# LowLevelAI/GLARE

Hardware: AMD Instinct MI355X
Metric: enhanced images/sec (400x600) (higher is better)
Workload: dtype fp16; 1 GPU; LOL eval15-shaped 400x600 inference, batch=8 per GPU, full encoder->flow->VQ->decoder->AFT (BASELINE configs[1]); batch_per_gpu=8, global_batch=8, input=3x400x600 (reflect-padded to 420x620), parallelism=dp1, streams_per_gpu=2, exchange=none (1 GPU), ranks_seen=1, weights=random, name-seeded (no checkpoints offline)

## Files before the change

glare_amd/csrc/conv_igemm_kernel.h:

```cpp
#pragma once
#include <type_traits>

#include "common.h"



struct ConvParams {
  const a16_t* in0;
  const a16_t* in1;
  const a16_t* wpk;
  const float* bias;
  const a16_t* res;
  void* out;
  int B, H, W;
  int IHs, IWs;
  int OH, OW;
  int Cin0, Cin1, CinTot;
  int p0, o0, p1, o1;
  int Cout, opitch, ooff, rpitch, roff;
  int upsample, act, out_mode;
  long long plane_pitch;
  int tiles_x, tiles_y, co_tiles, n_blocks, n_stages;
  int fast_epilogue;
  unsigned in0_bytes, in1_bytes;
  unsigned res_bytes;
  float* gn_part;
  int gn_nparts;
  const a16_t* res_lo;
  a16_t* out_lo;
  int groups, g_in_step, g_out_step, g_bias_step;
  long long g_w_elems;
  int k_wrap;
  const float* gn_coef;
  int gn_swish;
};

enum { EPI_FAST = 0,
       EPI_PLANAR = 1,
       EPI_GENERAL = 2 };
__host__ inline int conv_pick_epilogue(const ConvParams& p, bool planar_kernel) {
  const bool expk = p.act == GLARE_ACT_SIGMOID || p.act == GLARE_ACT_SWISH;
  if (p.out_mode == GLARE_OUT_NHWC_BF16 && p.fast_epilogue && !(p.res == nullptr && expk)) return EPI_FAST;
  if (planar_kernel && p.out_mode == GLARE_OUT_PLANAR_F32 && !p.res && !expk) return EPI_PLANAR;
  return EPI_GENERAL;
}

int glare_conv_launch_k3s1(const ConvParams& p, int tn, bool hilo, hipStream_t stream);
int glare_conv_launch_k3s1_planar(const ConvParams& p, int tn, hipStream_t stream);
int glare_conv_launch_k3s1_general(const ConvParams& p, int tn, hipStream_t stream);
int glare_conv_launch_k3s2(const ConvParams& p, int tn, bool hilo, hipStream_t stream);
int glare_conv_launch_k3s2_general(const ConvParams& p, int tn, hipStream_t stream);
int glare_conv_launch_k1(const ConvParams& p, int tn, bool hilo, hipStream_t stream);
int glare_conv_launch_k1_general(const ConvParams& p, int tn, hipStream_t stream);
int glare_conv_launch_k2(const ConvParams& p, int tn, hipStream_t stream);

namespace {

constexpr int TW = 32;



template <int KS, int STRIDE, int TH>
struct TileGeom {
  static constexpr int IH = (TH - 1) * STRIDE + KS;
  static constexpr int IW = (TW - 1) * STRIDE + KS;
  static constexpr int NPOS = IH * IW;
  static constexpr int PAD = (KS == 3 && STRIDE == 1) ? 1 : 0;
};

template <int N, typename F>
__device__ __forceinline__ void static_for(F&& f) {
  if constexpr (N > 0) {
    static_for<N - 1>(f);
    f(std::integral_constant<int, N - 1>{});
  }
}



__device__ __forceinline__ int fresh_lane_id() {
  int l;
  asm volatile("v_mbcnt_lo_u32_b32 %0, -1, 0\n\tv_mbcnt_hi_u32_b32 %0, -1, %0" : "=v"(l));
  return l;
}

__device__ __forceinline__ void gn_prologue_piece(u32x4* slot, const float* cf, int swish) {
  __builtin_amdgcn_sched_barrier(0);
  u32x4 v = *slot;
#pragma unroll
  for (int e = 0; e < 4; ++e) {
    const f32x4 q = *reinterpret_cast<const f32x4*>(cf + 4 * e);
    float lo = alo(v[e]) * q[0] + q[1];
    float hi = ahi(v[e]) * q[2] + q[3];
    if (swish) { lo = swishf_(lo); hi = swishf_(hi); }
    v[e] = pack_a2(lo, hi);
    __builtin_amdgcn_sched_barrier(0);
  }
  *slot = v;
  __builtin_amdgcn_sched_barrier(0);
}

template <int KS, int STRIDE, int MT, int NT, int WM, int WN, int KSTEPS, bool HILO = false, bool GNP = false, int EPI = EPI_FAST>
__global__ __launch_bounds__(64 * WM * WN, ((STRIDE == 1 && WM * WN == 4) ? 3 : 2)) void conv_igemm_kernel(const ConvParams p_in) {
  ConvParams p = p_in;
  if (p.groups > 1) {
    const int g = blockIdx.y;
    p.o0 += g * p.g_in_step;
    p.o1 += g * p.g_in_step;
    p.ooff += g * p.g_out_step;
    p.wpk += (size_t)g * p.g_w_elems;
    if (p.bias) p.bias += g * p.g_bias_step;
  }
  constexpr int TH = WM * MT;
  constexpr int NW = WM * WN;
  using G = TileGeom<KS, STRIDE, TH>;
  static_assert(NW == 4 || NW == 6 || NW == 8, "wave layout");
  constexpr int TN = WN * NT * 32;
  constexpr int A_CHUNKS = KSTEPS * 2 * G::NPOS;
  constexpr int A_INSTR = (A_CHUNKS + 63) / 64;
  constexpr int A_SLOTS = A_INSTR * 64;
  constexpr int A_PER_W = (A_INSTR + NW - 1) / NW;
  constexpr int B_CHUNKS = KS * KSTEPS * 2 * TN;
  static_assert(B_CHUNKS % 64 == 0, "B stage is a whole number of wave DMAs");
  constexpr int B_INSTR = B_CHUNKS / 64;
  constexpr int B_PER_W = (B_INSTR + NW - 1) / NW;
  constexpr int KC = 16 * KSTEPS;

  extern __shared__ __attribute__((aligned(16))) char smem[];
  u32x4* lA = reinterpret_cast<u32x4*>(smem);
  u32x4* lB = lA + 2 * A_SLOTS;

  int bid = blockIdx.x;
  {
    const int n = p.n_blocks, q = n / 8, r = n % 8, xcd = bid % 8, k = bid / 8;
    bid = (xcd < r ? xcd * (q + 1) : r * (q + 1) + (xcd - r) * q) + k;
  }
  const int ct = bid % p.co_tiles;
  int t = bid / p.co_tiles;
  int phase = 0;
  if (KS == 2) { phase = t & 3; t >>= 2; }
  const int pa = phase >> 1, pb = phase & 1;
  const int tx = t % p.tiles_x;
  t /= p.tiles_x;
  const int ty = t % p.tiles_y;
  const int b = t / p.tiles_y;

  const int tid = threadIdx.x, lane = tid & 63;
  const int wave = __builtin_amdgcn_readfirstlane(tid >> 6);
  const int wm = wave / WN, wn = wave % WN;
  const int oy0 = ty * TH, ox0 = tx * TW;
  const int iy0 = oy0 * STRIDE - G::PAD - (KS == 2 ? 1 - pa : 0), ix0 = ox0 * STRIDE - G::PAD - (KS == 2 ? 1 - pb : 0);

  f32x16 acc[MT][NT];
#pragma unroll
  for (int i = 0; i < MT; ++i)
#pragma unroll
    for (int j = 0; j < NT; ++j)
#pragma unroll
      for (int r = 0; r < 16; ++r) acc[i][j][r] = 0.f;

  constexpr unsigned A_OOB = 0x80000000u;
  unsigned a_vo0[A_PER_W], a_vo1[A_PER_W];
  int a_ck[A_PER_W];
#pragma unroll
  for (int i = 0; i < A_PER_W; ++i) {
    const int c = (wave + NW * i) * 64 + lane;
    a_vo0[i] = a_vo1[i] = A_OOB;
    a_ck[i] = 0;
    if (c < A_CHUNKS) {
      const int prow = c / (2 * KSTEPS * G::IW), rem = c % (2 * KSTEPS * G::IW);
      const int kk = rem / G::IW, pos = prow * G::IW + rem % G::IW;
      a_ck[i] = kk * 8;
      const int iy = iy0 + pos / G::IW, ix = ix0 + pos % G::IW;
      if (iy >= 0 && iy < p.IHs && ix >= 0 && ix < p.IWs) {
        const int sy = p.upsample ? (iy >> 1) : iy, sx = p.upsample ? (ix >> 1) : ix;
        const unsigned pix = (unsigned)(sy * p.W + sx);
        a_vo0[i] = (pix * (unsigned)p.p0 + (unsigned)(p.o0 + kk * 8)) * 2u;
        if constexpr (!GNP) a_vo1[i] = (pix * (unsigned)p.p1 + (unsigned)(p.o1 + kk * 8)) * 2u;
      }
    }
  }
  const size_t img = (size_t)b * p.H * p.W;
  const __amdgpu_buffer_rsrc_t arsrc0 =
      __builtin_amdgcn_make_buffer_rsrc(const_cast<a16_t*>(p.in0 + img * p.p0), 0, (int)p.in0_bytes, 0x00020000);
  const __amdgpu_buffer_rsrc_t arsrc1 = __builtin_amdgcn_make_buffer_rsrc(
      const_cast<a16_t*>(p.in1 ? p.in1 + img * p.p1 : p.in0), 0, (int)(p.in1 ? p.in1_bytes : p.in0_bytes), 0x00020000);
  const a16_t* wbase = p.wpk + ((size_t)phase * p.co_tiles + ct) * p.n_stages * (size_t)(KS * B_CHUNKS) * 8;

  const bool reuse = KS == 3 && !GNP && p.k_wrap == 2;
  const int n_pair = reuse ? 2 * (p.Cin0 / KC) : 0;
  auto a_is_new = [&](int stage) { return !(reuse && stage < n_pair && (stage & 1)); };
  auto issue_a = [&](int chunk, int buf, int i_lo = 0, int i_hi = 1 << 20) {
    const int c0 = chunk * KC;
    bool src0 = GNP || c0 < p.Cin0 || c0 >= p.Cin0 + p.Cin1;
    int cbase = c0 < p.Cin0 ? c0 : (src0 ? c0 - p.Cin0 - p.Cin1 : c0 - p.Cin0);
    if (reuse) {
      src0 = chunk < n_pair;
      cbase = src0 ? (chunk >> 1) * KC : (chunk - n_pair) * KC;
    }
    const int climit = src0 ? p.Cin0 : p.Cin1;
#pragma unroll
    for (int i = 0; i < A_PER_W; ++i) {
      const int j = wave + NW * i;
      if (i >= i_lo && i < i_hi && j < A_INSTR) {
        unsigned vo = src0 ? a_vo0[i] : a_vo1[i];
        if (cbase + a_ck[i] >= climit) vo = A_OOB;
        if (src0)
          __builtin_amdgcn_raw_ptr_buffer_load_lds(arsrc0, (__attribute__((address_space(3))) void*)(lA + buf * A_SLOTS + j * 64), 16, vo,
                                                   cbase * 2, 0, 0);
        else
          __builtin_amdgcn_raw_ptr_buffer_load_lds(arsrc1, (__attribute__((address_space(3))) void*)(lA + buf * A_SLOTS + j * 64), 16, vo,
                                                   cbase * 2, 0, 0);
      }
    }
  };
  const __amdgpu_buffer_rsrc_t wrsrc = __builtin_amdgcn_make_buffer_rsrc(
      const_cast<a16_t*>(wbase), 0, (int)((size_t)p.n_stages * KS * B_CHUNKS * 16), 0x00020000);
  const int lane16 = lane * 16;
  auto issue_b = [&](int bstage, int buf, int i_lo = 0, int i_hi = 1 << 20) {
#pragma unroll
    for (int i = 0; i < B_PER_W; ++i) {
      const int j = wave + NW * i;
      if (i >= i_lo && i < i_hi && j < B_INSTR)
        __builtin_amdgcn_raw_ptr_buffer_load_lds(wrsrc, (__attribute__((address_space(3))) void*)(lB + buf * B_CHUNKS + j * 64),
                                                 16, lane16, (bstage * B_CHUNKS + j * 64) * 16, 0, 0);
    }
  };

  [[maybe_unused]] auto prefetch_residual = [&](int free_buf) {
    if constexpr (KS == 3 && STRIDE == 1 && NW == 4 && TN == 128) {
      static_assert(A_SLOTS * 16 >= NW * 4 * 256, "room for the prefetch's landing zone");
      const size_t rimg = (size_t)b * p.OH * p.OW * p.rpitch;
#pragma unroll
      for (int k = 0; k < 2; ++k) {
        const int l = (wave * 2 + k) * 64 + lane;
        const int oy = oy0 + (l >> 6), ox = ox0 + ((l >> 1) & 31), co = ct * TN + (l & 1) * 64;
        const unsigned vo = (oy < p.OH && ox < p.OW && co < p.Cout)
                                ? (unsigned)(((oy * p.OW + ox) * p.rpitch + p.roff + co) * 2) : 0x80000000u;
        const __amdgpu_buffer_rsrc_t rr = __builtin_amdgcn_make_buffer_rsrc(const_cast<a16_t*>(p.res + rimg), 0, (int)p.res_bytes, 0x00020000);
        __builtin_amdgcn_raw_ptr_buffer_load_lds(rr, (__attribute__((address_space(3))) void*)(lA + free_buf * A_SLOTS + (wave * 4 + k) * 16),
                                                 4, vo, 0, 0, 0);
        if constexpr (HILO) {
          if (p.res_lo) {
            const __amdgpu_buffer_rsrc_t rl =
                __builtin_amdgcn_make_buffer_rsrc(const_cast<a16_t*>(p.res_lo + rimg), 0, (int)p.res_bytes, 0x00020000);
            __builtin_amdgcn_raw_ptr_buffer_load_lds(rl, (__attribute__((address_space(3))) void*)(lA + free_buf * A_SLOTS + (wave * 4 + 2 + k) * 16),
                                                     4, vo, 0, 0, 0);
          }
        }
      }
    }
  };

  [[maybe_unused]] float* lC = reinterpret_cast<float*>(lB + 2 * B_CHUNKS);
  [[maybe_unused]] auto gn_transform = [&](int chunk, int buf) {
    if constexpr (GNP) {
      const int c0 = chunk * KC;
#pragma unroll
      for (int i = 0; i < A_PER_W; ++i) {
        const int j = wave + NW * i;
        if (j < A_INSTR && a_vo0[i] != A_OOB && c0 + a_ck[i] < p.Cin0) {
          int ln = fresh_lane_id(), ck = a_ck[i];
          asm volatile("" : "+v"(ln), "+v"(ck));
          gn_prologue_piece(lA + buf * A_SLOTS + j * 64 + ln, lC + (c0 + ck) * 2, p.gn_swish);
        }
      }
    }
  };
  if constexpr (GNP) {
    const float* src = p.gn_coef + (size_t)b * p.Cin0 * 2;
    for (int i = tid; i < p.Cin0 * 2; i += 64 * NW) lC[i] = src[i];
    __syncthreads();
  }

  const int khalf = lane >> 5, px = lane & 31;
  const int n_bstages = p.n_stages * KS;
  issue_a(0, 0);
  issue_b(0, 0);
  int bs = 0;
  int a_cnt = 0;
  for (int chunk = 0; chunk < p.n_stages; ++chunk) {
    const u32x4* cA = lA + (a_cnt & 1) * A_SLOTS;
    const bool next_new = chunk + 1 < p.n_stages && a_is_new(chunk + 1);
#pragma unroll
    for (int trow = 0; trow < KS; ++trow, ++bs) {
      asm volatile("s_waitcnt vmcnt(0)" ::: "memory");
      if constexpr (GNP) {
        if (trow == 0 && chunk == 0) gn_transform(0, 0);
        if (trow == 1 && chunk + 1 < p.n_stages) gn_transform(chunk + 1, (a_cnt + 1) & 1);
      }
      __syncthreads();
      constexpr int NGRP = KS * KSTEPS;
      [[maybe_unused]] constexpr int B_PG = (B_PER_W + NGRP - 1) / NGRP, A_PG = (A_PER_W + NGRP - 1) / NGRP;
      const bool more_b = bs + 1 < n_bstages, more_a = trow == 0 && next_new;
      if (trow == 0 && chunk + 1 == p.n_stages && p.res_bytes) prefetch_residual((a_cnt + 1) & 1);
      const u32x4* cB = lB + (bs & 1) * B_CHUNKS;
#pragma unroll
      for (int tcol = 0; tcol < KS; ++tcol) {
#pragma unroll
        for (int ks = 0; ks < KSTEPS; ++ks) {
          {
            const int grp = tcol * KSTEPS + ks;
            if (more_b) issue_b(bs + 1, (bs + 1) & 1, grp * B_PG, (grp + 1) * B_PG);
            if (more_a) issue_a(chunk + 1, (a_cnt + 1) & 1, grp * A_PG, (grp + 1) * A_PG);
          }
          a16x8 bf[NT], af[MT];
#pragma unroll
          for (int j = 0; j < NT; ++j) {
            const int co = (wn * NT + j) * 32 + px;
            bf[j] = __builtin_bit_cast(a16x8, cB[((tcol * KSTEPS + ks) * 2 + khalf) * TN + co]);
          }
#pragma unroll
          for (int i = 0; i < MT; ++i) {
            const int row = wm * MT + i;
            af[i] = __builtin_bit_cast(a16x8, cA[((row * STRIDE + trow) * (2 * KSTEPS) + ks * 2 + khalf) * G::IW + px * STRIDE + tcol]);
          }
#pragma unroll
          for (int i = 0; i < MT; ++i)
#pragma unroll
            for (int j = 0; j < NT; ++j)
              acc[i][j] = mfma_a16_32x32x16(af[i], bf[j], acc[i][j], 0, 0, 0);
        }
      }
    }
    if (next_new) ++a_cnt;
  }

  if constexpr (HILO) {
    constexpr int ROWF = NT * 128 + 16;
    constexpr int CPR = NT * 4;
    static_assert(NW * 32 * ROWF <= (2 * A_SLOTS + 2 * B_CHUNKS) * 16, "hi/lo epilogue slab fits the pipeline LDS");
    static_assert(KS != 2, "the sub-pixel form has no hi/lo epilogue");
    __syncthreads();
    char* slab = smem + wave * (32 * ROWF);
    const int lane = fresh_lane_id();
    const int ncol = lane & 31, rhalf = lane >> 5;
    float gs0 = 0.f, gq0 = 0.f, gs1 = 0.f, gq1 = 0.f;
    const ActSel asel = act_sel(p.act);
    static_for<MT>([&](auto ic) {
      constexpr int i = decltype(ic)::value;
      static_for<NT>([&](auto jc) {
        constexpr int j = decltype(jc)::value;
        const int co = ct * TN + (wn * NT + j) * 32 + ncol;
        const float bv = (p.bias && co < p.Cout) ? p.bias[co] : 0.f;
#pragma unroll
        for (int r = 0; r < 16; ++r) {
          const int m = (r & 3) + 8 * (r >> 2) + 4 * rhalf;
          *reinterpret_cast<float*>(slab + m * ROWF + (j * 32 + ncol) * 4) = acc[i][j][r] + bv;
        }
      });
      constexpr int NIT = 32 * CPR / 64;
      [[maybe_unused]] u32x4 rvv[NIT], rlv[NIT];
      const bool res_buf = p.res && p.res_bytes;
      __builtin_amdgcn_sched_barrier(0);
      if (res_buf) {
        const size_t rimg = (size_t)b * p.OH * p.OW * p.rpitch;
        const __amdgpu_buffer_rsrc_t rr = __builtin_amdgcn_make_buffer_rsrc(const_cast<a16_t*>(p.res + rimg), 0, (int)p.res_bytes, 0x00020000);
        const __amdgpu_buffer_rsrc_t rl = __builtin_amdgcn_make_buffer_rsrc(const_cast<a16_t*>((p.res_lo ? p.res_lo : p.res) + rimg), 0,
                                                                            (int)p.res_bytes, 0x00020000);
        const int oy = oy0 + wm * MT + i;
        const unsigned vo = oy < p.OH ? (unsigned)((((oy * p.OW + ox0 + lane / CPR) * p.rpitch) + p.roff + ct * TN + wn * NT * 32 + (lane % CPR) * 8) * 2)
                                      : 0x80000000u;
#pragma unroll
        for (int it = 0; it < NIT; ++it) {
          const unsigned o = vo + (unsigned)(it * (64 / CPR) * p.rpitch * 2);
          rvv[it] = __builtin_amdgcn_raw_buffer_load_b128(rr, o, 0, 0);
          if (p.res_lo) rlv[it] = __builtin_amdgcn_raw_buffer_load_b128(rl, o, 0, 0);
        }
      }
      asm volatile("s_waitcnt lgkmcnt(0)" ::: "memory");
#pragma unroll
      for (int it = 0; it < NIT; ++it) {
        const int idx = lane + 64 * it;
        const int row = idx / CPR, ch = idx % CPR;
        const int oy = oy0 + wm * MT + i, ox = ox0 + row;
        const int co = ct * TN + wn * NT * 32 + ch * 8;
        if (oy < p.OH && ox < p.OW && co < p.Cout) {
          const f32x4 f0 = *reinterpret_cast<const f32x4*>(slab + row * ROWF + ch * 32);
          const f32x4 f1 = *reinterpret_cast<const f32x4*>(slab + row * ROWF + ch * 32 + 16);
          float v[8] = {f0[0], f0[1], f0[2], f0[3], f1[0], f1[1], f1[2], f1[3]};
          const size_t pix = ((size_t)b * p.OH + oy) * p.OW + ox;
          if (p.res) {
            const u32x4 rv = res_buf ? rvv[it] : *reinterpret_cast<const u32x4*>(p.res + pix * p.rpitch + p.roff + co);
#pragma unroll
            for (int e = 0; e < 4; ++e) { v[2 * e] += alo(rv[e]); v[2 * e + 1] += ahi(rv[e]); }
            if (p.res_lo) {
              const u32x4 rl = res_buf ? rlv[it] : *reinterpret_cast<const u32x4*>(p.res_lo + pix * p.rpitch + p.roff + co);
#pragma unroll
              for (int e = 0; e < 4; ++e) { v[2 * e] += alo(rl[e]); v[2 * e + 1] += ahi(rl[e]); }
            }
          }
          if (asel.expk) {
#pragma unroll
            for (int e = 0; e < 8; ++e) v[e] = act_exp(v[e], asel.expk);
          } else {
#pragma unroll
            for (int e = 0; e < 8; ++e) v[e] = act_cheap(v[e], asel.relu);
          }
          u32x4 hi, lo;
#pragma unroll
          for (int e = 0; e < 4; ++e) {
            const float a = v[2 * e], c = v[2 * e + 1];
            hi[e] = pack_a2(a, c);
            lo[e] = pack_a2(a - alo(hi[e]), c - ahi(hi[e]));
            if (e < 2) { gs0 += a + c; gq0 += a * a + c * c; } else { gs1 += a + c; gq1 += a * a + c * c; }
          }
          *reinterpret_cast<u32x4*>(reinterpret_cast<a16_t*>(p.out) + pix * p.opitch + p.ooff + co) = hi;
          *reinterpret_cast<u32x4*>(p.out_lo + pix * p.opitch + p.ooff + co) = lo;
        }
      }
      asm volatile("s_waitcnt lgkmcnt(0)" ::: "memory");
    });
    if (p.gn_part) {
#pragma unroll
      for (int o = CPR; o < 64; o <<= 1) {
        gs0 += __shfl_xor(gs0, o, 64); gq0 += __shfl_xor(gq0, o, 64);
        gs1 += __shfl_xor(gs1, o, 64); gq1 += __shfl_xor(gq1, o, 64);
      }
      const int co = ct * TN + wn * NT * 32 + lane * 8;
      if (lane < CPR && co < p.Cout) {
        const int row0 = oy0 + wm * MT;
        const int part = ((phase * ((p.OH + 7) / 8) + row0 / 8) * p.tiles_x + tx) * 2 + ((row0 / 4) & 1);
        if (part < p.gn_nparts) {
          float* dst = p.gn_part + (((size_t)b * p.gn_nparts + part) * (p.Cout / 4) + co / 4) * 2;
          dst[0] = gs0; dst[1] = gq0; dst[2] = gs1; dst[3] = gq1;
        }
      }
    }
    return;
  }

  if constexpr (EPI == EPI_FAST) {
    constexpr int HT = (NW == 8 || MT < 2) ? 1 : MT / 2;
    constexpr int HROWS = HT * 32;
    constexpr int ROWB = NT * 64 + 16;
    constexpr int CPR = NT * 4;
    static_assert(NW * HROWS * ROWB <= (2 * A_SLOTS + 2 * B_CHUNKS) * 16, "epilogue slab fits the pipeline LDS");
    __syncthreads();
    char* slab = smem + wave * (HROWS * ROWB);
    const int lane = fresh_lane_id();
    const int ncol = lane & 31, rhalf = lane >> 5, odd = lane & 1;
    const bool act_early = p.res == nullptr;
    float gs0 = 0.f, gq0 = 0.f, gs1 = 0.f, gq1 = 0.f;
    const ActSel asel = act_sel(p.act);
    const bool relu_early = act_early && asel.relu;
    static_for<MT / HT>([&](auto hc) {
      constexpr int half = decltype(hc)::value;
      static_for<NT>([&](auto jc) {
        constexpr int j = decltype(jc)::value;
        const int co = ct * TN + (wn * NT + j) * 32 + ncol;
        const float bv = (p.bias && co < p.Cout) ? p.bias[co] : 0.f;
        static_for<HT>([&](auto ic) {
          constexpr int il = decltype(ic)::value;
#pragma unroll
          for (int t = 0; t < 8; ++t) {
            constexpr int i = half * HT + il;
            const float a = act_cheap(acc[i][j][2 * t] + bv, relu_early), c = act_cheap(acc[i][j][2 * t + 1] + bv, relu_early);
            const float send = odd ? a : c;
            const float recv = __shfl_xor(send, 1, 64);
            const int r = 2 * t + odd;
            const int m = (r & 3) + 8 * (r >> 2) + 4 * rhalf;
            const uint32_t w = odd ? pack_a2(recv, c) : pack_a2(a, recv);
            *reinterpret_cast<uint32_t*>(slab + (il * 32 + m) * ROWB + (j * 32 + (ncol & ~1)) * 2) = w;
          }
        });
      });
      constexpr int NIT = HROWS * CPR / 64;
      constexpr bool RES_AHEAD = NIT <= 8 && KS != 2;
      [[maybe_unused]] u32x4 rvv[RES_AHEAD ? NIT : 1];
      bool res_buf = false;
      if constexpr (RES_AHEAD) {
        res_buf = p.res && p.res_bytes;
        __builtin_amdgcn_sched_barrier(0);
        if (res_buf) {
          const size_t rimg = (size_t)b * p.OH * p.OW * p.rpitch;
          const __amdgpu_buffer_rsrc_t rr = __builtin_amdgcn_make_buffer_rsrc(const_cast<a16_t*>(p.res + rimg), 0, (int)p.res_bytes, 0x00020000);
          const int oyb = oy0 + wm * MT + half * HT;
          const unsigned vo = (unsigned)((((oyb * p.OW + ox0 + lane / CPR) * p.rpitch) + p.roff + ct * TN + wn * NT * 32 + (lane % CPR) * 8) * 2);
#pragma unroll
          for (int it = 0; it < NIT; ++it) {
            constexpr int RPI = 64 / CPR;
            const int dy = (it * RPI) / 32, dx = (it * RPI) % 32;
            const unsigned o = oyb + dy < p.OH ? vo + (unsigned)((dy * p.OW + dx) * p.rpitch * 2) : 0x80000000u;
            rvv[it] = __builtin_amdgcn_raw_buffer_load_b128(rr, o, 0, 0);
          }
        }
      }
      asm volatile("s_waitcnt lgkmcnt(0)" ::: "memory");
#pragma unroll
      for (int it = 0; it < NIT; ++it) {
        const int idx = lane + 64 * it;
        const int row = idx / CPR, ch = idx % CPR;
        const int oy = oy0 + wm * MT + half * HT + row / 32, ox = ox0 + (row & 31);
        const int co = ct * TN + wn * NT * 32 + ch * 8;
        if (oy < p.OH && ox < p.OW && co < p.Cout) {
          u32x4 v = *reinterpret_cast<const u32x4*>(slab + row * ROWB + ch * 16);
          const size_t pix = KS == 2 ? ((size_t)b * (2 * p.OH) + 2 * oy + pa) * (size_t)(2 * p.OW) + 2 * ox + pb
                                     : ((size_t)b * p.OH + oy) * p.OW + ox;
          if (p.res) {
            u32x4 rv;
            if (res_buf) rv = rvv[RES_AHEAD ? it : 0];
            else rv = *reinterpret_cast<const u32x4*>(p.res + pix * p.rpitch + p.roff + co);
            if (asel.expk) {
#pragma unroll
              for (int e = 0; e < 4; ++e) v[e] = pack_a2(act_exp(alo(v[e]) + alo(rv[e]), asel.expk), act_exp(ahi(v[e]) + ahi(rv[e]), asel.expk));
            } else {
#pragma unroll
              for (int e = 0; e < 4; ++e) v[e] = pack_a2(act_cheap(alo(v[e]) + alo(rv[e]), asel.relu), act_cheap(ahi(v[e]) + ahi(rv[e]), asel.relu));
            }
          }
          *reinterpret_cast<u32x4*>(reinterpret_cast<a16_t*>(p.out) + pix * p.opitch + p.ooff + co) = v;
          if (p.gn_part) {
#pragma unroll
            for (int e = 0; e < 2; ++e) {
              const float x0 = alo(v[e]), x1 = ahi(v[e]), y0 = alo(v[2 + e]), y1 = ahi(v[2 + e]);
              gs0 += x0 + x1; gq0 += x0 * x0 + x1 * x1;
              gs1 += y0 + y1; gq1 += y0 * y0 + y1 * y1;
            }
          }
        }
      }
      asm volatile("s_waitcnt lgkmcnt(0)" ::: "memory");
    });
    if (p.gn_part) {
#pragma unroll
      for (int o = CPR; o < 64; o <<= 1) {
        gs0 += __shfl_xor(gs0, o, 64); gq0 += __shfl_xor(gq0, o, 64);
        gs1 += __shfl_xor(gs1, o, 64); gq1 += __shfl_xor(gq1, o, 64);
      }
      const int co = ct * TN + wn * NT * 32 + lane * 8;
      if (lane < CPR && co < p.Cout) {
        const int row0 = oy0 + wm * MT;
        const int part = ((phase * ((p.OH + 7) / 8) + row0 / 8) * p.tiles_x + tx) * 2 + ((row0 / 4) & 1);
        if (part < p.gn_nparts) {
          float* dst = p.gn_part + (((size_t)b * p.gn_nparts + part) * (p.Cout / 4) + co / 4) * 2;
          dst[0] = gs0; dst[1] = gq0; dst[2] = gs1; dst[3] = gq1;
        }
      }
    }
    return;
  }

  if constexpr (EPI == EPI_PLANAR) {
    static_assert(!HILO && KS == 3 && STRIDE == 1 && NW == 4, "the planar slab epilogue exists for the 3x3 stride-1 4-wave kernels");
    {
      constexpr int ROWD = NT * 32 + 1;
      static_assert(NW * 32 * ROWD * 4 <= (2 * A_SLOTS + 2 * B_CHUNKS) * 16, "planar epilogue slab fits the pipeline LDS");
      typedef float f32x4u __attribute__((ext_vector_type(4), aligned(4)));
      __syncthreads();
      float* slab = reinterpret_cast<float*>(smem) + wave * (32 * ROWD);
      const int lane = fresh_lane_id();
      const int ncol = lane & 31, rhalf = lane >> 5;
      const ActSel asel = act_sel(p.act);
      static_for<MT>([&](auto ic) {
        constexpr int i = decltype(ic)::value;
        static_for<NT>([&](auto jc) {
          constexpr int j = decltype(jc)::value;
          const int co = ct * TN + (wn * NT + j) * 32 + ncol;
          const float bv = (p.bias && co < p.Cout) ? p.bias[co] : 0.f;
#pragma unroll
          for (int r = 0; r < 16; ++r) {
            const int m = (r & 3) + 8 * (r >> 2) + 4 * rhalf;
            slab[m * ROWD + j * 32 + ncol] = act_cheap(acc[i][j][r] + bv, asel.relu);
          }
        });
        asm volatile("s_waitcnt lgkmcnt(0)" ::: "memory");
        const int oy = oy0 + wm * MT + i;
#pragma unroll
        for (int it = 0; it < 8 * NT * 32 / 64; ++it) {
          const int idx = lane + 64 * it;
          const int q = idx & 7, cl = idx >> 3;
          const int co = ct * TN + wn * NT * 32 + cl, x0 = ox0 + 4 * q;
          if (oy < p.OH && co < p.Cout && x0 < p.OW) {
            const f32x4u v = {slab[(4 * q) * ROWD + cl], slab[(4 * q + 1) * ROWD + cl], slab[(4 * q + 2) * ROWD + cl],
                              slab[(4 * q + 3) * ROWD + cl]};
            float* dst = reinterpret_cast<float*>(p.out) + ((size_t)b * p.opitch + p.ooff + co) * (size_t)p.plane_pitch + (size_t)oy * p.OW + x0;
            if (x0 + 3 < p.OW) {
              *reinterpret_cast<f32x4u*>(dst) = v;
            } else {
#pragma unroll
              for (int e = 0; e < 4; ++e)
                if (x0 + e < p.OW) dst[e] = v[e];
            }
          }
        }
        asm volatile("s_waitcnt lgkmcnt(0)" ::: "memory");
      });
      return;
    }
  }

  if constexpr (EPI == EPI_GENERAL) {
  const int lane = fresh_lane_id();
  const int ncol = lane & 31, rhalf = lane >> 5;
  const ActSel asel = act_sel(p.act);
  static_for<NT>([&](auto jc) {
    constexpr int j = decltype(jc)::value;
    const int co = ct * TN + (wn * NT + j) * 32 + ncol;
    const bool co_ok = co < p.Cout;
    const float bv = (co_ok && p.bias) ? p.bias[co] : 0.f;
    static_for<MT>([&](auto ic) {
      constexpr int i = decltype(ic)::value;
      const int oy = oy0 + wm * MT + i;
      const bool row_ok = oy < p.OH;
#pragma unroll
      for (int rq = 0; rq < 4; ++rq) {
        const int xb = ox0 + 8 * rq + 4 * rhalf;
        float v[4];
#pragma unroll
        for (int e = 0; e < 4; ++e) v[e] = acc[i][j][rq * 4 + e] + bv;
        const size_t pix0 = ((size_t)b * p.OH + oy) * p.OW + xb;
        if (p.out_mode == GLARE_OUT_NHWC_BF16 || p.out_mode == GLARE_OUT_NHWC_F32) {
#pragma unroll
          for (int e = 0; e < 4; ++e) {
            if (row_ok && co_ok && xb + e < p.OW) {
              float y = v[e];
              if (p.res) y += a2f(p.res[(pix0 + e) * p.rpitch + p.roff + co]);
              y = act_any(y, asel);
              if (p.out_mode == GLARE_OUT_NHWC_BF16)
                reinterpret_cast<a16_t*>(p.out)[(pix0 + e) * p.opitch + p.ooff + co] = f2a(y);
              else
                reinterpret_cast<float*>(p.out)[(pix0 + e) * p.opitch + p.ooff + co] = y;
            }
          }
        } else {
          if (co_ok && row_ok) {
            const size_t base = ((size_t)b * p.opitch + p.ooff + co) * (size_t)p.plane_pitch + (size_t)oy * p.OW + xb;
#pragma unroll
            for (int e = 0; e < 4; ++e) {
              if (xb + e < p.OW) {
                const float y = act_any(v[e], asel);
                if (p.out_mode == GLARE_OUT_PLANAR_F32)
                  reinterpret_cast<float*>(p.out)[base + e] = y;
                else
                  reinterpret_cast<a16_t*>(p.out)[base + e] = f2a(y);
              }
            }
          }
        }
      }
    });
  });
  }
}

template <int KS, int STRIDE, int MT, int NT, int WM, int WN, int KSTEPS, bool HILO = false, bool GNP = false, int EPI = EPI_FAST>
int launch(const ConvParams& p_in, hipStream_t stream) {
  using G = TileGeom<KS, STRIDE, WM * MT>;
  constexpr int TN = WN * NT * 32;
  ConvParams p = p_in;
  p.tiles_y = cdiv(p.OH, WM * MT);
  const long long nb = (long long)p.B * p.tiles_x * p.tiles_y * p.co_tiles * (KS == 2 ? 4 : 1);
  if (nb > 0x7fffffffLL) return GLARE_ERR_INVALID;
  p.n_blocks = (int)nb;
  p.gn_nparts = p.tiles_x * cdiv(p.OH, 8) * 2 * (KS == 2 ? 4 : 1);
  if (p.gn_part && !(p.fast_epilogue && p.Cout % 32 == 0)) return GLARE_ERR_UNSUPPORTED;
  if (p.gn_part && !HILO && EPI != EPI_FAST) return GLARE_ERR_UNSUPPORTED;
  const size_t lds = (size_t)(2 * (((KSTEPS * 2 * G::NPOS + 63) / 64) * 64) + 2 * KS * KSTEPS * 2 * TN) * 16 + (GNP ? (size_t)p.Cin0 * 8 : 0);
  constexpr bool PLANAR_KERNEL = !HILO && KS == 3 && STRIDE == 1 && WM * WN == 4;
  if (!HILO && conv_pick_epilogue(p, PLANAR_KERNEL) != EPI) return GLARE_ERR_INVALID;
  auto kern = conv_igemm_kernel<KS, STRIDE, MT, NT, WM, WN, KSTEPS, HILO, GNP, EPI>;
  if (lds > 64 * 1024 &&
      hipFuncSetAttribute((const void*)kern, hipFuncAttributeMaxDynamicSharedMemorySize, (int)lds) != hipSuccess)
    return GLARE_ERR_LAUNCH;
  hipLaunchKernelGGL(kern, dim3(p.n_blocks, p.groups > 1 ? p.groups : 1), dim3(64 * WM * WN), lds, stream, p);
  return glare_launch_status();
}

}
```

Before: 64.67 images/sec.

## Swap MFMA operands so accumulators hold channel quads, vectorize conv epilogues

Swaps the A/B operands of the 32x32x16 MFMA so each lane's accumulator registers hold four consecutive output channels for one pixel instead of four pixels for one channel. Every epilogue (hi/lo, fast NHWC, planar, general) is rewritten for this transposed layout: bias is loaded as float4 quads staged in the LDS slab pad, the shuffle-xor pairing is dropped in favour of packed 64-bit slab writes with an XOR swizzle undone on readback, and the general path gets vectorized NHWC stores. It also reloads ConvParams from the kernarg segment after the main loop to reduce register pressure across it. The change is broad and touches layout invariants in several epilogues, so any indexing mismatch would produce wrong outputs.

```diff
diff --git a/glare_amd/csrc/conv_igemm_kernel.h b/glare_amd/csrc/conv_igemm_kernel.h
--- a/glare_amd/csrc/conv_igemm_kernel.h
+++ b/glare_amd/csrc/conv_igemm_kernel.h
@@ -84,6 +84,26 @@
   return l;
 }
 
+typedef float f32x4u __attribute__((ext_vector_type(4), aligned(4)));
+template <bool WHOLE = false>
+__device__ __forceinline__ f32x4 bias_quad(const float* bias, int co, int Cout) {
+  f32x4 q = {0.f, 0.f, 0.f, 0.f};
+  if (bias) {
+    if constexpr (WHOLE) {
+      const f32x4 v = *reinterpret_cast<const f32x4u*>(bias + (co < Cout ? co : 0));
+#pragma unroll
+      for (int e = 0; e < 4; ++e) q[e] = co < Cout ? v[e] : 0.f;
+    } else if (co + 3 < Cout) {
+      q = *reinterpret_cast<const f32x4u*>(bias + co);
+    } else {
+#pragma unroll
+      for (int e = 0; e < 4; ++e)
+        if (co + e < Cout) q[e] = bias[co + e];
+    }
+  }
+  return q;
+}
+
 __device__ __forceinline__ void gn_prologue_piece(u32x4* slot, const float* cf, int swish) {
   __builtin_amdgcn_sched_barrier(0);
   u32x4 v = *slot;
@@ -107,9 +127,11 @@
     const int g = blockIdx.y;
     p.o0 += g * p.g_in_step;
     p.o1 += g * p.g_in_step;
-    p.ooff += g * p.g_out_step;
     p.wpk += (size_t)g * p.g_w_elems;
-    if (p.bias) p.bias += g * p.g_bias_step;
+    if constexpr (GNP) {
+      p.ooff += g * p.g_out_step;
+      if (p.bias) p.bias += g * p.g_bias_step;
+    }
   }
   constexpr int TH = WM * MT;
   constexpr int NW = WM * WN;
@@ -319,11 +341,19 @@
           for (int i = 0; i < MT; ++i)
 #pragma unroll
             for (int j = 0; j < NT; ++j)
-              acc[i][j] = mfma_a16_32x32x16(af[i], bf[j], acc[i][j], 0, 0, 0);
+              acc[i][j] = mfma_a16_32x32x16(bf[j], af[i], acc[i][j], 0, 0, 0);
         }
       }
     }
     if (next_new) ++a_cnt;
+  }
+  const ConvParams& p_entry = p;
+  {
+  ConvParams p = p_entry;
+  if constexpr (!GNP) {
+    p = *(const ConvParams*)__builtin_amdgcn_kernarg_segment_ptr();
+    p.ooff += blockIdx.y * p.g_out_step;
+    if (p.bias) p.bias += blockIdx.y * p.g_bias_step;
   }
 
   if constexpr (HILO) {
@@ -334,20 +364,25 @@
     __syncthreads();
     char* slab = smem + wave * (32 * ROWF);
     const int lane = fresh_lane_id();
-    const int ncol = lane & 31, rhalf = lane >> 5;
+    const int xl = lane & 31, rhalf = lane >> 5;
     float gs0 = 0.f, gq0 = 0.f, gs1 = 0.f, gq1 = 0.f;
     const ActSel asel = act_sel(p.act);
+    static_assert(NT * 8 <= 32, "one bias quad per slab row pad");
+    {
+      const int q = lane & (NT * 8 - 1);
+      *reinterpret_cast<f32x4*>(slab + q * ROWF + NT * 128) = bias_quad<true>(p.bias, ct * TN + wn * NT * 32 + 4 * q, p.Cout);
+    }
+    asm volatile("s_waitcnt lgkmcnt(0)" ::: "memory");
     static_for<MT>([&](auto ic) {
       constexpr int i = decltype(ic)::value;
       static_for<NT>([&](auto jc) {
         constexpr int j = decltype(jc)::value;
-        const int co = ct * TN + (wn * NT + j) * 32 + ncol;
-        const float bv = (p.bias && co < p.Cout) ? p.bias[co] : 0.f;
-#pragma unroll
-        for (int r = 0; r < 16; ++r) {
-          const int m = (r & 3) + 8 * (r >> 2) + 4 * rhalf;
-          *reinterpret_cast<float*>(slab + m * ROWF + (j * 32 + ncol) * 4) = acc[i][j][r] + bv;
-        }
+        static_for<4>([&](auto gc) {
+          constexpr int g = decltype(gc)::value;
+          const f32x4 bq = *reinterpret_cast<const f32x4*>(slab + (j * 8 + 2 * g + rhalf) * ROWF + NT * 128);
+          const f32x4 v = {acc[i][j][4 * g] + bq[0], acc[i][j][4 * g + 1] + bq[1], acc[i][j][4 * g + 2] + bq[2], acc[i][j][4 * g + 3] + bq[3]};
+          *reinterpret_cast<f32x4*>(slab + xl * ROWF + (j * 32 + 8 * g + 4 * rhalf) * 4) = v;
+        });
       });
       constexpr int NIT = 32 * CPR / 64;
       [[maybe_unused]] u32x4 rvv[NIT], rlv[NIT];
@@ -439,7 +474,14 @@
     __syncthreads();
     char* slab = smem + wave * (HROWS * ROWB);
     const int lane = fresh_lane_id();
-    const int ncol = lane & 31, rhalf = lane >> 5, odd = lane & 1;
+    const int xl = lane & 31, rhalf = lane >> 5;
+    const int wofs = xl * ROWB + 8 * (rhalf ^ ((xl >> 3) & 1));
+    static_assert(NT * 8 <= HROWS, "one bias quad per slab row pad");
+    {
+      const int q = lane & (NT * 8 - 1);
+      *reinterpret_cast<f32x4*>(slab + q * ROWB + NT * 64) = bias_quad<true>(p.bias, ct * TN + wn * NT * 32 + 4 * q, p.Cout);
+    }
+    asm volatile("s_waitcnt lgkmcnt(0)" ::: "memory");
     const bool act_early = p.res == nullptr;
     float gs0 = 0.f, gq0 = 0.f, gs1 = 0.f, gq1 = 0.f;
     const ActSel asel = act_sel(p.act);
@@ -448,21 +490,16 @@
       constexpr int half = decltype(hc)::value;
       static_for<NT>([&](auto jc) {
         constexpr int j = decltype(jc)::value;
-        const int co = ct * TN + (wn * NT + j) * 32 + ncol;
-        const float bv = (p.bias && co < p.Cout) ? p.bias[co] : 0.f;
-        static_for<HT>([&](auto ic) {
-          constexpr int il = decltype(ic)::value;
-#pragma unroll
-          for (int t = 0; t < 8; ++t) {
+        static_for<4>([&](auto gc) {
+          constexpr int g = decltype(gc)::value;
+          const f32x4 bq = *reinterpret_cast<const f32x4*>(slab + (j * 8 + 2 * g + rhalf) * ROWB + NT * 64);
+          static_for<HT>([&](auto ic) {
+            constexpr int il = decltype(ic)::value;
             constexpr int i = half * HT + il;
-            const float a = act_cheap(acc[i][j][2 * t] + bv, relu_early), c = act_cheap(acc[i][j][2 * t + 1] + bv, relu_early);
-            const float send = odd ? a : c;
-            const float recv = __shfl_xor(send, 1, 64);
-            const int r = 2 * t + odd;
-            const int m = (r & 3) + 8 * (r >> 2) + 4 * rhalf;
-            const uint32_t w = odd ? pack_a2(recv, c) : pack_a2(a, recv);
-            *reinterpret_cast<uint32_t*>(slab + (il * 32 + m) * ROWB + (j * 32 + (ncol & ~1)) * 2) = w;
-          }
+            const u32x2 w = {pack_a2(act_cheap(acc[i][j][4 * g] + bq[0], relu_early), act_cheap(acc[i][j][4 * g + 1] + bq[1], relu_early)),
+                             pack_a2(act_cheap(acc[i][j][4 * g + 2] + bq[2], relu_early), act_cheap(acc[i][j][4 * g + 3] + bq[3], relu_early))};
+            *reinterpret_cast<u32x2*>(slab + il * 32 * ROWB + wofs + j * 64 + g * 16) = w;
+          });
         });
       });
       constexpr int NIT = HROWS * CPR / 64;
@@ -495,6 +532,11 @@
         const int co = ct * TN + wn * NT * 32 + ch * 8;
         if (oy < p.OH && ox < p.OW && co < p.Cout) {
           u32x4 v = *reinterpret_cast<const u32x4*>(slab + row * ROWB + ch * 16);
+          {
+            const uint32_t m = (row & 8) ? 0xffffffffu : 0u;
+            const uint32_t t0 = (v[0] ^ v[2]) & m, t1 = (v[1] ^ v[3]) & m;
+            v[0] ^= t0; v[2] ^= t0; v[1] ^= t1; v[3] ^= t1;
+          }
           const size_t pix = KS == 2 ? ((size_t)b * (2 * p.OH) + 2 * oy + pa) * (size_t)(2 * p.OW) + 2 * ox + pb
                                      : ((size_t)b * p.OH + oy) * p.OW + ox;
           if (p.res) {
@@ -544,25 +586,28 @@
   if constexpr (EPI == EPI_PLANAR) {
     static_assert(!HILO && KS == 3 && STRIDE == 1 && NW == 4, "the planar slab epilogue exists for the 3x3 stride-1 4-wave kernels");
     {
-      constexpr int ROWD = NT * 32 + 1;
-      static_assert(NW * 32 * ROWD * 4 <= (2 * A_SLOTS + 2 * B_CHUNKS) * 16, "planar epilogue slab fits the pipeline LDS");
-      typedef float f32x4u __attribute__((ext_vector_type(4), aligned(4)));
+      constexpr int CHP = 32;
+      constexpr int SLABD = NW * NT * 32 * CHP;
+      static_assert((SLABD + NW * NT * 32) * 4 <= (2 * A_SLOTS + 2 * B_CHUNKS) * 16, "planar epilogue slab fits the pipeline LDS");
       __syncthreads();
-      float* slab = reinterpret_cast<float*>(smem) + wave * (32 * ROWD);
+      float* slab = reinterpret_cast<float*>(smem) + wave * (NT * 32 * CHP);
+      float* lbias = reinterpret_cast<float*>(smem) + SLABD + wave * (NT * 32);
       const int lane = fresh_lane_id();
-      const int ncol = lane & 31, rhalf = lane >> 5;
+      const int xl = lane & 31, rhalf = lane >> 5;
       const ActSel asel = act_sel(p.act);
+      if (lane < NT * 8) *reinterpret_cast<f32x4*>(lbias + 4 * lane) = bias_quad(p.bias, ct * TN + wn * NT * 32 + 4 * lane, p.Cout);
+      asm volatile("s_waitcnt lgkmcnt(0)" ::: "memory");
       static_for<MT>([&](auto ic) {
         constexpr int i = decltype(ic)::value;
         static_for<NT>([&](auto jc) {
           constexpr int j = decltype(jc)::value;
-          const int co = ct * TN + (wn * NT + j) * 32 + ncol;
-          const float bv = (p.bias && co < p.Cout) ? p.bias[co] : 0.f;
-#pragma unroll
-          for (int r = 0; r < 16; ++r) {
-            const int m = (r & 3) + 8 * (r >> 2) + 4 * rhalf;
-            slab[m * ROWD + j * 32 + ncol] = act_cheap(acc[i][j][r] + bv, asel.relu);
-          }
+          static_for<4>([&](auto gc) {
+            constexpr int g = decltype(gc)::value;
+            const int cl = j * 32 + 8 * g + 4 * rhalf;
+            const f32x4 bq = *reinterpret_cast<const f32x4*>(lbias + cl);
+#pragma unroll
+            for (int e = 0; e < 4; ++e) slab[(cl + e) * CHP + xl] = act_cheap(acc[i][j][4 * g + e] + bq[e], asel.relu);
+          });
         });
         asm volatile("s_waitcnt lgkmcnt(0)" ::: "memory");
         const int oy = oy0 + wm * MT + i;
@@ -572,8 +617,7 @@
           const int q = idx & 7, cl = idx >> 3;
           const int co = ct * TN + wn * NT * 32 + cl, x0 = ox0 + 4 * q;
           if (oy < p.OH && co < p.Cout && x0 < p.OW) {
-            const f32x4u v = {slab[(4 * q) * ROWD + cl], slab[(4 * q + 1) * ROWD + cl], slab[(4 * q + 2) * ROWD + cl],
-                              slab[(4 * q + 3) * ROWD + cl]};
+            const f32x4 v = *reinterpret_cast<const f32x4*>(slab + cl * CHP + 4 * q);
             float* dst = reinterpret_cast<float*>(p.out) + ((size_t)b * p.opitch + p.ooff + co) * (size_t)p.plane_pitch + (size_t)oy * p.OW + x0;
             if (x0 + 3 < p.OW) {
               *reinterpret_cast<f32x4u*>(dst) = v;
@@ -592,55 +636,71 @@
 
   if constexpr (EPI == EPI_GENERAL) {
   const int lane = fresh_lane_id();
-  const int ncol = lane & 31, rhalf = lane >> 5;
+  const int xl = lane & 31, rhalf = lane >> 5;
   const ActSel asel = act_sel(p.act);
+  const bool nhwc = p.out_mode == GLARE_OUT_NHWC_BF16 || p.out_mode == GLARE_OUT_NHWC_F32;
+  const bool out16 = p.out_mode == GLARE_OUT_NHWC_BF16;
+  const bool vec = nhwc && !((p.opitch | p.ooff) & 3) && !(reinterpret_cast<uintptr_t>(p.out) & (out16 ? 7 : 15)) &&
+                   (!p.res || (!((p.rpitch | p.roff) & 3) && !(reinterpret_cast<uintptr_t>(p.res) & 7)));
+  const int ox = ox0 + xl;
   static_for<NT>([&](auto jc) {
     constexpr int j = decltype(jc)::value;
-    const int co = ct * TN + (wn * NT + j) * 32 + ncol;
-    const bool co_ok = co < p.Cout;
-    const float bv = (co_ok && p.bias) ? p.bias[co] : 0.f;
-    static_for<MT>([&](auto ic) {
-      constexpr int i = decltype(ic)::value;
-      const int oy = oy0 + wm * MT + i;
-      const bool row_ok = oy < p.OH;
-#pragma unroll
-      for (int rq = 0; rq < 4; ++rq) {
-        const int xb = ox0 + 8 * rq + 4 * rhalf;
-        float v[4];
-#pragma unroll
-        for (int e = 0; e < 4; ++e) v[e] = acc[i][j][rq * 4 + e] + bv;
-        const size_t pix0 = ((size_t)b * p.OH + oy) * p.OW + xb;
-        if (p.out_mode == GLARE_OUT_NHWC_BF16 || p.out_mode == GLARE_OUT_NHWC_F32) {
-#pragma unroll
-          for (int e = 0; e < 4; ++e) {
-            if (row_ok && co_ok && xb + e < p.OW) {
-              float y = v[e];
-              if (p.res) y += a2f(p.res[(pix0 + e) * p.rpitch + p.roff + co]);
-              y = act_any(y, asel);
-              if (p.out_mode == GLARE_OUT_NHWC_BF16)
-                reinterpret_cast<a16_t*>(p.out)[(pix0 + e) * p.opitch + p.ooff + co] = f2a(y);
+    static_for<4>([&](auto gc) {
+      constexpr int g = decltype(gc)::value;
+      const int co = ct * TN + (wn * NT + j) * 32 + 8 * g + 4 * rhalf;
+      const f32x4 bq = bias_quad(p.bias, co, p.Cout);
+      static_for<MT>([&](auto ic) {
+        constexpr int i = decltype(ic)::value;
+        const int oy = oy0 + wm * MT + i;
+        if (oy < p.OH && ox < p.OW && co < p.Cout) {
+          float v[4];
+#pragma unroll
+          for (int e = 0; e < 4; ++e) v[e] = acc[i][j][4 * g + e] + bq[e];
+          if (nhwc) {
+            const size_t pix = ((size_t)b * p.OH + oy) * p.OW + ox;
+            if (vec && co + 3 < p.Cout) {
+              if (p.res) {
+                const u32x2 rv = *reinterpret_cast<const u32x2*>(p.res + pix * p.rpitch + p.roff + co);
+                v[0] += alo(rv[0]); v[1] += ahi(rv[0]); v[2] += alo(rv[1]); v[3] += ahi(rv[1]);
+              }
+#pragma unroll
+              for (int e = 0; e < 4; ++e) v[e] = act_any(v[e], asel);
+              if (out16)
+                *reinterpret_cast<u32x2*>(reinterpret_cast<a16_t*>(p.out) + pix * p.opitch + p.ooff + co) = u32x2{pack_a2(v[0], v[1]), pack_a2(v[2], v[3])};
               else
-                reinterpret_cast<float*>(p.out)[(pix0 + e) * p.opitch + p.ooff + co] = y;
+                *reinterpret_cast<f32x4*>(reinterpret_cast<float*>(p.out) + pix * p.opitch + p.ooff + co) = f32x4{v[0], v[1], v[2], v[3]};
+            } else {
+#pragma unroll
+              for (int e = 0; e < 4; ++e) {
+                if (co + e < p.Cout) {
+                  float y = v[e];
+                  if (p.res) y += a2f(p.res[pix * p.rpitch + p.roff + co + e]);
+                  y = act_any(y, asel);
+                  if (out16)
+                    reinterpret_cast<a16_t*>(p.out)[pix * p.opitch + p.ooff + co + e] = f2a(y);
+                  else
+                    reinterpret_cast<float*>(p.out)[pix * p.opitch + p.ooff + co + e] = y;
+                }
+              }
             }
-          }
-        } else {
-          if (co_ok && row_ok) {
-            const size_t base = ((size_t)b * p.opitch + p.ooff + co) * (size_t)p.plane_pitch + (size_t)oy * p.OW + xb;
+          } else {
 #pragma unroll
             for (int e = 0; e < 4; ++e) {
-              if (xb + e < p.OW) {
+              if (co + e < p.Cout) {
+                const size_t at = ((size_t)b * p.opitch + p.ooff + co + e) * (size_t)p.plane_pitch + (size_t)oy * p.OW + ox;
                 const float y = act_any(v[e], asel);
                 if (p.out_mode == GLARE_OUT_PLANAR_F32)
-                  reinterpret_cast<float*>(p.out)[base + e] = y;
+                  reinterpret_cast<float*>(p.out)[at] = y;
                 else
-                  reinterpret_cast<a16_t*>(p.out)[base + e] = f2a(y);
+                  reinterpret_cast<a16_t*>(p.out)[at] = f2a(y);
               }
             }
           }
         }
-      }
+      });
     });
   });
+  }
   }
 }
 
```

Measured after the change: 64.91 images/sec, median of 6. Within noise of the previous version (+0.4%).
